# SysCV/LiDAR_snow_sim

Hardware: NVIDIA H100
Metric: augmented LiDAR points/sec (higher is better)
Workload: dtype f64

## Files before the change

### lidar_snow_sim_b200/csrc/solve.cu

```cuda
#include "beam.cuh"

namespace {

constexpr int SOLVE_TPB = 128;
constexpr int SOLVE_WARPS = SOLVE_TPB / 32;
#ifndef LSS_SOLVE_CTAS
#define LSS_SOLVE_CTAS 6
#endif
#ifndef LSS_SOLVE_ARENA
#define LSS_SOLVE_ARENA 160
#endif
constexpr int SOLVE_CTAS_PER_SM = LSS_SOLVE_CTAS;
constexpr int ARENA = LSS_SOLVE_ARENA;
constexpr int SOLVE_LCAP = 128;
static_assert(SOLVE_LCAP + 1 <= ARENA, "a beam with SOLVE_LCAP occluders must fit a round of the arena on its own");
constexpr unsigned FULL = 0xffffffffu;

struct Beam {
    double d, right, left;
    bool straddle;
};

__device__ __forceinline__ void beam_limits(float th32, double half_div, Beam &bm)
{
    const double thd = (double)th32;
    double right = thd - half_div, left = thd + half_div;
    if (right < 0) right += LSS_TWO_PI;
    if (left < 0) left += LSS_TWO_PI;
    if (right > LSS_TWO_PI) right -= LSS_TWO_PI;
    if (left > LSS_TWO_PI) left -= LSS_TWO_PI;
    bm.right = right; bm.left = left; bm.straddle = right > left;
}

__device__ __forceinline__ bool exact_hit(const ParticleRec *rp, const Beam &bm, double &rho, bool &right_hit, bool &left_hit)
{
    rho = rp->rho;
    if (!(rho < bm.d)) return false;
    const double phi = rp->phi, alpha = rp->alpha;
    bool inside = (bm.right <= phi) && (phi <= bm.left);
    if (bm.straddle) inside = inside || ((bm.right - LSS_TWO_PI <= phi) && (phi <= bm.left)) ||
                              ((bm.right <= phi) && (phi <= bm.left + LSS_TWO_PI));
    right_hit = within(bm.right - phi, alpha);
    left_hit = within(bm.left - phi, alpha);
    return inside || right_hit || left_hit;
}

struct Bucket {
    int e0, e1;
    float th_rel;
    long long pbase;
};

__device__ __forceinline__ Bucket beam_bucket(const DevArgs &a, int plane, float th32)
{
    const double thd = (double)th32;
    const double thm = thd >= LSS_TWO_PI ? thd - LSS_TWO_PI : thd;
    int bk = (int)(thm * a.inv_w);
    bk = bk < 0 ? 0 : (bk >= a.n_buckets ? a.n_buckets - 1 : bk);
    const int32_t *bs = a.bucket_start + (int64_t)plane * (a.n_buckets + 1) + bk;
    Bucket k;
    k.e0 = bs[0];
    k.e1 = bs[1];
    k.th_rel = (float)(thm - (bk + 0.5) * a.w);
    k.pbase = a.plane_off[plane];
    return k;
}

template <class F>
__device__ __forceinline__ int for_each_hit(const DevArgs &a, const Bucket &k, const Beam &bm, float d32, F &&f)
{
    int n = 0;
#pragma unroll 1
    for (int e = k.e0; e < k.e1; e++) {
        const EntryView en = lss_decode(__ldg(&a.entries[e]), a.zbase);
        if (!(en.x < d32)) break;
        if (!(fabsf(en.y - k.th_rel) <= en.z)) continue;
        const long long pi = k.pbase + en.idx;
        double rho;
        bool rh, lh;
        if (exact_hit(a.rec + pi, bm, rho, rh, lh)) { f((int)pi, rho, rh, lh); n++; }
    }
    return n;
}

constexpr int SURV_CAP = 20;

__device__ __forceinline__ double shfl_f64(double v, int src)
{
    const long long b = __double_as_longlong(v);
    const int lo = __shfl_sync(FULL, (int)(unsigned)b, src), hi = __shfl_sync(FULL, (int)(b >> 32), src);
    return __longlong_as_double(((long long)hi << 32) | (unsigned)lo);
}

#ifndef LSS_SCAN_CTAS
#define LSS_SCAN_CTAS 10
#endif
__global__ void __launch_bounds__(SNOW_TPB, LSS_SCAN_CTAS) k_scan(DevArgs a)
{
    __shared__ float s_rows[SNOW_WARPS][32 * 5];
    __shared__ int s_idx[SNOW_WARPS][32][SURV_CAP];
    __shared__ unsigned s_hit[SNOW_WARPS][32];
    const int lane = threadIdx.x & 31, wid = threadIdx.x >> 5;
    const int st = blockIdx.x * SNOW_WARPS + wid;
    if (st >= a.n_wtiles) return;
    const unsigned long long se = a.sched[st];
    const int b = (int)((se >> 32) & 0xffffu), w0 = (int)(unsigned)se;
    const int64_t beg = a.cloud_off[b];
    const int n = (int)(a.cloud_off[b + 1] - beg);
    const int i = w0 + lane;
    const bool active = i < n;
    const int nf_w = min(32, n - w0) * 5;
    float px = 0, py = 0, pz = 0, pint = 0, pch = 0;
    {
        const float *src = a.pts + (beg + w0) * 5;
#pragma unroll
        for (int q = 0; q < 5; q++) {
            const int f = q * 32 + lane;
            if (f < nf_w) s_rows[wid][f] = __ldcs(src + f);
        }
        __syncwarp();
        if (active) {
            const float *row = &s_rows[wid][5 * lane];
            px = row[0]; py = row[1]; pz = row[2]; pint = row[3]; pch = row[4];
        }
    }
    const float d32 = __fsqrt_rn(__fadd_rn(__fadd_rn(__fmul_rn(px, px), __fmul_rn(py, py)), __fmul_rn(pz, pz)));
    const int ch = channel_bin(pch);
    float out_l = pch;
    int ns = 0;
    Bucket bkt;
    bkt.e0 = bkt.e1 = 0; bkt.th_rel = 0.0f; bkt.pbase = 0;
    bool slow = false;
    float th32 = 0.0f;
    Beam bm;
    bm.d = (double)d32; bm.right = bm.left = 0.0; bm.straddle = false;
    if (active && ch < LSS_N_CHANNELS) {
        out_l = 0.0f;
        th32 = a.theta ? a.theta[beg + i] : azimuth32(py, px);
        if (th32 < 0.0f) th32 = __fadd_rn(th32, 6.2831855f);
        beam_limits(th32, a.half_div, bm);
        const int plane = a.order[b * LSS_N_CHANNELS + ch];
        if (plane >= 0 && plane < a.n_planes && th32 == th32) {
            bkt = beam_bucket(a, plane, th32);
            const int e1 = bkt.e1;
            int *pos = s_idx[wid][lane];
            bool stop = false;
#pragma unroll 1
            for (int e = bkt.e0; e < e1 && !stop; e += 4) {
                BroadEntry raw[4];
#pragma unroll
                for (int q = 0; q < 4; q++) raw[q] = __ldg(&a.entries[min(e + q, e1 - 1)]);
#pragma unroll
                for (int q = 0; q < 4; q++) {
                    if (stop || e + q >= e1) continue;
                    const EntryView en = lss_decode(raw[q], a.zbase);
                    if (!(en.x < d32)) { stop = true; continue; }
                    if (!(fabsf(en.y - bkt.th_rel) <= en.z)) continue;
                    if (ns < SURV_CAP) pos[ns] = en.idx;
                    else slow = true;
                    ns++;
                }
            }
        }
    }
    s_hit[wid][lane] = 0u;
    const int mine = slow ? 0 : ns;
    int incl = mine;
#pragma unroll
    for (int sft = 1; sft < 32; sft <<= 1) {
        const int t = __shfl_up_sync(FULL, incl, sft);
        if (lane >= sft) incl += t;
    }
    const int off = incl - mine;
    const int total = __shfl_sync(FULL, incl, 31);
    __syncwarp();
#pragma unroll 1
    for (int s0 = 0; s0 < total; s0 += 32) {
        const int s = s0 + lane;
        int j = 0;
#pragma unroll
        for (int step = 16; step; step >>= 1) {
            const int c = j + step;
            const int oc = __shfl_sync(FULL, off, c & 31);
            if (c < 32 && oc <= s) j = c;
        }
        const int r = s - __shfl_sync(FULL, off, j);
        const long long pbj = __shfl_sync(FULL, bkt.pbase, j);
        Beam bj;
        bj.d = shfl_f64(bm.d, j);
        bj.right = shfl_f64(bm.right, j);
        bj.left = shfl_f64(bm.left, j);
        bj.straddle = bj.right > bj.left;
        if (s < total) {
            double rho;
            bool rh, lh;
            if (exact_hit(a.rec + pbj + s_idx[wid][j][r], bj, rho, rh, lh)) atomicOr(&s_hit[wid][j], 1u << r);
        }
    }
    __syncwarp();
    unsigned hits = s_hit[wid][lane];
    int L = __popc(hits);
    if (slow) L = for_each_hit(a, bkt, bm, d32, [](int, double, bool, bool) {});
    {
        const bool push = L > 0;
        const unsigned pm = __ballot_sync(FULL, push);
        int lincl = push ? L : 0;
#pragma unroll
        for (int sft = 1; sft < 32; sft <<= 1) {
            const int t = __shfl_up_sync(FULL, lincl, sft);
            if (lane >= sft) lincl += t;
        }
        const int ltotal = __shfl_sync(FULL, lincl, 31);
        if (pm) {
            int hbase = 0;
            const int leader = __ffs(pm) - 1;
            if (lane == leader) hbase = atomicAdd(a.hdr + 2, ltotal);
            hbase = __shfl_sync(FULL, hbase, leader);
            if (push) {
                const int cls = LIST_CLASSES - 1 - min(LIST_CLASSES - 1, 2 * min(L, 63) + (d32 > 40.0f ? 1 : 0));
                const unsigned cm = __match_any_sync(pm, cls);
                const int cl = __ffs(cm) - 1;
                int j = 0;
                if (lane == cl) j = atomicAdd(a.hdr + LIST_CLASSES + cls, __popc(cm));
                j = __shfl_sync(cm, j, cl) + __popc(cm & ((1u << lane) - 1u));
                int *ct = a.chunk_tab + (int64_t)cls * a.chunks_per_class + j / LIST_CHUNK;
                if (j % LIST_CHUNK == 0) atomicExch(ct, atomicAdd(a.hdr, 1) + 1);
                __syncwarp(pm);
                int chunk;
                while ((chunk = *(volatile int *)ct) == 0) {}
                const int hoff = hbase + lincl - L;
                const bool fits = hoff + L <= a.hit_cap;
                {
                    SolveItem it;
                    it.key = ((unsigned long long)ch << 56) | ((unsigned long long)cls << 48) |
                             ((unsigned long long)b << 32) | (unsigned)i;
                    it.hit_off = fits ? hoff : -1;
                    it.L = L;
                    it.th32 = th32;
                    it.px = px;
                    it.py = py;
                    it.pz = pz;
                    a.items[(int64_t)(chunk - 1) * LIST_CHUNK + j % LIST_CHUNK] = it;
                }
                if (fits) {
                    int *hp = a.hit_idx + hoff;
                    if (!slow) {
                        const int *pos = s_idx[wid][lane];
#pragma unroll 1
                        for (int k = 0; hits; hits &= hits - 1) hp[k++] = (int)bkt.pbase + pos[__ffs(hits) - 1];
                    } else {
                        for_each_hit(a, bkt, bm, d32, [&](int pi, double, bool, bool) { *hp++ = pi; });
                    }
                }
            }
        }
    }
    __syncwarp();
    if (active) {
        float *row = &s_rows[wid][5 * lane];
        const float out_i = rintf(pint);
        row[3] = out_i;
        row[4] = out_l;
        if (a.nocc) a.nocc[beg + i] = 0;
        a.keep_d[beg + i] = d32;
        a.keep_i[beg + i] = out_i;
        a.keep_tag[beg + i] = (uint8_t)ch;
    }
    __syncwarp();
    {
        float *dst = a.aug + (beg + w0) * 5;
#pragma unroll
        for (int q = 0; q < 5; q++) {
            const int f = q * 32 + lane;
            if (f < nf_w) dst[f] = s_rows[wid][f];
        }
    }
}

__device__ __forceinline__ unsigned long long pack_win(int ks, int ke, int k0)
{
    return (unsigned long long)(unsigned)ks | ((unsigned long long)(unsigned)ke << 11) | ((unsigned long long)(unsigned)k0 << 22);
}

__device__ __forceinline__ void pulse_phase(double r, double &sb, double &cb)
{
    const double ctau = 299792458.0 * 1e-8, inv_ctau = 1.0 / (299792458.0 * 1e-8);
    const double bh = r * inv_ctau;
    const double bl = fma(-bh, ctau, r) * inv_ctau;
    double s, c;
    sincospi(bh, &s, &c);
    const double corr = LSS_PI * bl;
    sb = fma(corr, c, s);
    cb = fma(-corr, s, c);
}

__global__ void __launch_bounds__(SOLVE_TPB, SOLVE_CTAS_PER_SM) k_solve(DevArgs a, int *tile_cursor)
{
    __shared__ double s_arena[SOLVE_WARPS][4][ARENA];
    __shared__ unsigned long long s_piece[SOLVE_WARPS][2 * ARENA];
    __shared__ int s_piece_k[SOLVE_WARPS][2 * ARENA];
    const int lane = threadIdx.x & 31, wid = threadIdx.x >> 5;
    unsigned long long *PD = s_piece[wid];
    int *PK = s_piece_k[wid];
    double *A0 = s_arena[wid][0], *A1 = s_arena[wid][1], *A2 = s_arena[wid][2], *A3 = s_arena[wid][3];
    unsigned long long *W = reinterpret_cast<unsigned long long *>(A2);

    __shared__ int s_tile0[LIST_CLASSES + 1];
    const int *cls_cnt = a.hdr + LIST_CLASSES;
    if (wid == 0) {
        int run = 0;
        for (int c0 = 0; c0 < LIST_CLASSES; c0 += 32) {
            const int v = (cls_cnt[c0 + lane] + 31) >> 5;
            int incl = v;
#pragma unroll
            for (int sft = 1; sft < 32; sft <<= 1) {
                const int t = __shfl_up_sync(FULL, incl, sft);
                if (lane >= sft) incl += t;
            }
            s_tile0[c0 + lane] = run + incl - v;
            run += __shfl_sync(FULL, incl, 31);
        }
        if (lane == 0) s_tile0[LIST_CLASSES] = run;
    }
    __syncthreads();
    const int n_tiles = s_tile0[LIST_CLASSES];
    const double ctau = 299792458.0 * 1e-8;
    const double inv_step = (double)(LSS_M_EXT - 1) / (120 + ctau);

    for (;;) {
        int tile = 0;
        if (lane == 0) tile = atomicAdd(tile_cursor, 1);
        tile = __shfl_sync(FULL, tile, 0);
        if (tile >= n_tiles) break;
        int cls = 0;
#pragma unroll
        for (int step = LIST_CLASSES / 2; step; step >>= 1)
            if (s_tile0[cls + step] <= tile) cls += step;
        const int j = (tile - s_tile0[cls]) * 32 + lane;
        const bool active = j < cls_cnt[cls];
        SolveItem it;
        it.key = 0ull; it.hit_off = 0; it.L = 0; it.th32 = 0.0f; it.px = 0.0f; it.py = 0.0f; it.pz = 0.0f;
        if (active) {
            const int chunk = a.chunk_tab[(int64_t)cls * a.chunks_per_class + j / LIST_CHUNK];
            it = a.items[(int64_t)(chunk - 1) * LIST_CHUNK + j % LIST_CHUNK];
        }
        const int b = (int)((it.key >> 32) & 0xffffu);
        const int i = (int)(it.key & 0xffffffffu);
        const int ch = (int)(it.key >> 56);
        const int64_t beg = a.cloud_off[b];
        const float px = it.px, py = it.py, pz = it.pz;
        const float d32 = __fsqrt_rn(__fadd_rn(__fadd_rn(__fmul_rn(px, px), __fmul_rn(py, py)), __fmul_rn(pz, pz)));

        float out_x = px, out_y = py, out_z = pz, out_i = 0.0f, out_l = 0.0f;
        long long att_new_i = -1;
        int n_claim = 0;

        const int L = active ? it.L : 0;
        Beam bm;
        bm.d = (double)d32;
        beam_limits(it.th32, a.half_div, bm);

        if (L > SOLVE_LCAP) raise_status(a.status, LSS_ERR_OCCLUDER_OVERFLOW);
        const int need = (L > 0 && L <= SOLVE_LCAP) ? L + 1 : 0;

        unsigned remaining = __ballot_sync(FULL, need > 0);
        while (remaining) {
            const bool rem = (remaining >> lane) & 1u;
            const int mine = rem ? need : 0;
            int incl = mine;
#pragma unroll
            for (int s = 1; s < 32; s <<= 1) {
                const int t = __shfl_up_sync(FULL, incl, s);
                if (lane >= s) incl += t;
            }
            const bool in_round = rem && incl <= ARENA;
            remaining &= ~__ballot_sync(FULL, in_round);
            const int off = incl - mine;
            const int total = (int)__reduce_max_sync(FULL, in_round ? (unsigned)incl : 0u);
            int n_pulses = 0;
            double amax = 0.0;
            double best = 0.0;
            int kbest = 0;

#pragma unroll 1
            for (int s0 = 0; s0 < total; s0 += 32) {
                const int s = s0 + lane;
                int j = 0;
#pragma unroll
                for (int step = 16; step; step >>= 1) {
                    const int c = j + step;
                    const int oc = __shfl_sync(FULL, off, c & 31);
                    if (c < 32 && oc <= s) j = c;
                }
                const int r = s - __shfl_sync(FULL, off, j);
                const int Lj = __shfl_sync(FULL, L, j);
                const int hoj = __shfl_sync(FULL, it.hit_off, j);
                const int inr = __shfl_sync(FULL, (int)in_round, j);
                Beam bj;
                bj.d = shfl_f64(bm.d, j);
                bj.right = shfl_f64(bm.right, j);
                bj.left = shfl_f64(bm.left, j);
                bj.straddle = bj.right > bj.left;
                if (s < total && inr && r < Lj && hoj >= 0) {
                    const int pi = a.hit_idx[hoj + r];
                    const ParticleTan tn = a.tan[pi];
                    double rho;
                    bool rh, lh;
                    exact_hit(a.rec + pi, bj, rho, rh, lh);
                    A0[s] = rh ? bj.right : tn.t_right;
                    A1[s] = lh ? bj.left : tn.t_left;
                    A2[s] = rho;
                }
            }
            if (in_round && it.hit_off < 0) {
                const Bucket bkt = beam_bucket(a, a.order[b * LSS_N_CHANNELS + ch], it.th32);
                int s = off;
                for_each_hit(a, bkt, bm, d32, [&](int pi, double rho, bool rh, bool lh) {
                    A0[s] = rh ? bm.right : a.tan[pi].t_right;
                    A1[s] = lh ? bm.left : a.tan[pi].t_left;
                    A2[s] = rho;
                    s++;
                });
            }
            __syncwarp();

            if (in_round) {
#pragma unroll 1
                for (int p = 1; p < L; p++) {
                    const double rho = A2[off + p];
                    if (!(A2[off + p - 1] > rho)) continue;
                    const double a1 = A0[off + p], a2 = A1[off + p];
                    int q = p - 1;
#pragma unroll 1
                    while (q >= 0 && A2[off + q] > rho) { A0[off + q + 1] = A0[off + q]; A1[off + q + 1] = A1[off + q]; A2[off + q + 1] = A2[off + q]; q--; }
                    A0[off + q + 1] = a1; A1[off + q + 1] = a2; A2[off + q + 1] = rho;
                }

                double rb = bm.right;
                if (bm.straddle) rb = bm.right - LSS_TWO_PI;
                int nu = 0, P = 0;
                double ep_min = fmin(rb, bm.left), ep_max = fmax(rb, bm.left), claimed_total = 0.0;
#pragma unroll 1
                for (int j = 0; j < L; j++) {
                    double lo = A0[off + j];
                    const double hi = A1[off + j], rho = A2[off + j];
                    if (bm.straddle && lo > hi) lo -= LSS_TWO_PI;
                    ep_min = fmin(ep_min, fmin(lo, hi));
                    ep_max = fmax(ep_max, fmax(lo, hi));
                    if (!(lo < hi)) continue;
                    bool contained = false;
                    double cov = 0.0, nlo = lo, nhi = hi;
                    int w = 0;
#pragma unroll 1
                    for (int u = 0; u < nu; u++) {
                        const double ul = A0[off + u], uh = A1[off + u];
                        if ((ul <= lo) && (hi <= uh)) { contained = true; break; }
                        if (ul <= hi && uh >= lo) {
                            const double ov = fmin(hi, uh) - fmax(lo, ul);
                            if (ov > 0.0) cov += ov;
                            nlo = fmin(nlo, ul);
                            nhi = fmax(nhi, uh);
                        } else {
                            A0[off + w] = ul; A1[off + w] = uh; w++;
                        }
                    }
                    if (contained) continue;
                    const double claimed = (hi - lo) - cov;
                    claimed_total += claimed;
                    A0[off + w] = nlo; A1[off + w] = nhi;
                    nu = w + 1;
                    double ratio = claimed / a.div_rad;
                    ratio = ratio < 0 ? 0 : (ratio > 1 ? 1 : ratio);
                    A2[off + P] = rho;
                    A3[off + P] = ratio;
                    P++;
                }
                n_claim = P;
                double ratio_hard = ((ep_max - ep_min) - claimed_total) / a.div_rad;
                ratio_hard = ratio_hard < 0 ? 0 : (ratio_hard > 1 ? 1 : ratio_hard);

                if (P > 0) {
                    const double beta_0 = 1 * 1e-06 / LSS_PI;
                    const double i_orig = 0.9 * a.sensor->max_intensity[ch];
                    const double A = (i_orig / beta_0) * beta_0;
                    bool bad = false;
#pragma unroll 1
                    for (int j = 0; j < P; j++) {
                        const double r = A2[off + j], ratio = A3[off + j];
                        const int ks = (int)ceil(r * 10);
                        const int ke = (int)(floor((r + ctau) * 10) + 1);
                        bad |= (ke > LSS_M_EXT) || (ks < 0);
                        double sb, cb;
                        pulse_phase(r, sb, cb);
                        const double amp = (A * ratio * xsi64(r)) / (r * r);
                        amax = fmax(amax, amp);
                        A0[off + j] = amp;
                        A1[off + j] = sb;
                        A3[off + j] = cb;
                        W[off + j] = pack_win(ks, ke, (int)rint((r + ctau / 2) * inv_step));
                    }
                    {
                        const int ks = (int)ceilf(__fmul_rn(d32, 10.0f));
                        const int ke = (int)(floorf(__fmul_rn(__fadd_rn(d32, (float)ctau), 10.0f)) + 1.0f);
                        bad |= (ke > LSS_M_EXT) || (ks < 0);
                        double sb, cb;
                        pulse_phase(bm.d, sb, cb);
                        const double amp = (A * ratio_hard * xsi32(d32)) / (double)__fmul_rn(d32, d32);
                        amax = fmax(amax, amp);
                        A0[off + P] = amp;
                        A1[off + P] = sb;
                        A3[off + P] = cb;
                        W[off + P] = pack_win(ks, ke, (int)rint((bm.d + ctau / 2) * inv_step));
                    }
                    if (bad) raise_status(a.status, LSS_ERR_RANGE_INDEX);
                    else n_pulses = P + 1;
                }
            }

            int np_mine = 0;
            if (n_pulses > 0) {
                const double lb = 0.99 * amax;
                double asum = 0.0;
                int qa = 0, qb = -1, nxt = 0;
                int ks_n = (int)(W[off] & 2047u);
                int ke_a = 0;
                int k = ks_n;
                unsigned long long *pd = PD + 2 * off;
#pragma unroll 1
                for (;;) {
#pragma unroll 1
                    while (ks_n <= k) {
                        qb = nxt++;
                        asum += A0[off + qb];
                        ks_n = nxt < n_pulses ? (int)(W[off + nxt] & 2047u) : 4096;
                    }
#pragma unroll 1
                    while (qa <= qb) {
                        ke_a = (int)((W[off + qa] >> 11) & 2047u);
                        if (ke_a > k) break;
                        asum -= A0[off + qa];
                        qa++;
                    }
                    if (qa > qb) {
                        asum = 0.0;
                        if (nxt >= n_pulses) break;
                        k = ks_n;
                        continue;
                    }
                    const int pend = min(ke_a, ks_n);
                    if (asum * 1.0001 >= lb)
                        pd[np_mine++] = (unsigned long long)(unsigned)k | ((unsigned long long)(unsigned)pend << 11) |
                                        ((unsigned long long)(unsigned)(off + qa) << 22) | ((unsigned long long)(unsigned)(off + qb) << 32);
                    k = pend;
                }
            }
            int pincl = np_mine;
#pragma unroll
            for (int sft = 1; sft < 32; sft <<= 1) {
                const int t = __shfl_up_sync(FULL, pincl, sft);
                if (lane >= sft) pincl += t;
            }
            const int pex = pincl - np_mine;
            const int ptotal = __shfl_sync(FULL, pincl, 31);
            __syncwarp();
            {
                const float step = (float)((120 + ctau) / (double)(LSS_M_EXT - 1));
                const float ctau_f = (float)ctau;
#pragma unroll 1
                for (int f0 = 0; f0 < ptotal; f0 += 32) {
                    const int f = f0 + lane;
                    int j = 0;
#pragma unroll
                    for (int stp = 16; stp; stp >>= 1) {
                        const int c = j + stp;
                        const int oc = __shfl_sync(FULL, pex, c & 31);
                        if (c < 32 && oc <= f) j = c;
                    }
                    const int slot = 2 * __shfl_sync(FULL, off, j) + (f - __shfl_sync(FULL, pex, j));
                    if (f < ptotal) {
                        const unsigned long long d = PD[slot];
                        const int lo = (int)(d & 2047u), hi = (int)((d >> 11) & 2047u);
                        const int qa = (int)((d >> 22) & 1023u), qb = (int)((d >> 32) & 1023u);
                        double pbest = 0.0;
                        int pk = lo;
                        auto eval = [&](int c) {
                            const double2 t = __ldg(&a.wtab[c]);
                            double v = 0.0;
#pragma unroll 1
                            for (int q = qa; q <= qb; q++) {
                                const double sn = t.x * A3[q] - t.y * A1[q];
                                v += A0[q] * (sn * sn);
                            }
                            if (v > pbest) { pbest = v; pk = c; }
                        };
                        int kc;
                        bool all = false;
                        if (qa == qb) {
                            kc = (int)((W[qa] >> 22) & 2047u);
                        } else {
                            float zx = 0.0f, zy = 0.0f, asum = 0.0f;
#pragma unroll 1
                            for (int q = qa; q <= qb; q++) {
                                const float A = (float)A0[q], sn = (float)A1[q], cs = (float)A3[q];
                                zx += A * (cs * cs - sn * sn);
                                zy += A * (2.0f * sn * cs);
                                asum += A;
                            }
                            all = zx * zx + zy * zy < 1e-6f * asum * asum;
                            const float r0 = (atan2f(zy, zx) + 3.14159265f) * (ctau_f * 0.15915494f);
                            const float rc = 0.5f * (float)(lo + hi - 1) * step;
                            kc = (int)rintf((r0 + rintf((rc - r0) / ctau_f) * ctau_f) / step);
                        }
                        const int c_lo = all ? lo : max(lo, min(hi - 1, kc - 1));
                        const int c_hi = all ? hi - 1 : min(hi - 1, max(lo, kc + 1));
#pragma unroll 1
                        for (int c = c_lo; c <= c_hi; c++) eval(c);
                        PD[slot] = (unsigned long long)__double_as_longlong(pbest);
                        PK[slot] = pk;
                    }
                }
            }
            __syncwarp();
#pragma unroll 1
            for (int r = 0; r < np_mine; r++) {
                const double v = __longlong_as_double((long long)PD[2 * off + r]);
                if (v > best) { best = v; kbest = PK[2 * off + r]; }
            }
            __syncwarp();

            if (n_pulses > 0) {
                const double max_i = a.sensor->max_intensity[ch];
                const double min_i = a.sensor->min_intensity[ch];
                const double d_max = ((double)kbest / 10) - (ctau / 2);
                const double q1 = 1 - d_max / 120;
                double i_max = best + max_i * a.sensor->focal_slope[ch] * fabs(a.sensor->focal_offset[ch] - q1 * q1);
                i_max = i_max < min_i ? min_i : (i_max > max_i ? max_i : i_max);
                const long long new_i = (long long)i_max;
                if (fabs(d_max - bm.d) < 2 * (1.0 / 10)) {
                    out_l = 1.0f;
                    att_new_i = new_i;
                } else {
                    out_l = 2.0f;
                    const double sc = d_max / bm.d;
                    out_x = (float)((double)px * sc);
                    out_y = (float)((double)py * sc);
                    out_z = (float)((double)pz * sc);
                }
                if (new_i < 0) raise_status(a.status, LSS_ERR_NEGATIVE_INTENSITY);
                double ci = (double)new_i;
                ci = ci < min_i ? min_i : (ci > max_i ? max_i : ci);
                out_i = (float)ci;
            }
            __syncwarp();
        }

        if (active) {
            if (out_l != 0.0f) {
                const float ri = rintf(out_i);
                float *row = a.aug + (beg + i) * 5;
                row[0] = out_x; row[1] = out_y; row[2] = out_z; row[3] = ri; row[4] = out_l;
                a.keep_i[beg + i] = ri;
                a.keep_tag[beg + i] = keep_tag_of(ch, out_l);
            }
            if (a.nocc) a.nocc[beg + i] = n_claim;
        }
        {
            const bool on = att_new_i >= 0;
            const int key = b * LSS_N_CHANNELS + (ch < LSS_N_CHANNELS ? ch : 0);
            const unsigned mk = __match_any_sync(FULL, on ? key : -1);
            if (on && lane == __ffs(mk) - 1) atomicAdd(a.att_cnt + key, (unsigned)__popc(mk));
            const unsigned mb = __match_any_sync(FULL, on ? b : -1);
            const unsigned sum = __reduce_add_sync(mb, on ? (unsigned)att_new_i : 0u);
            if (on && lane == __ffs(mb) - 1) atomicAdd(&a.att_sum[b], (unsigned long long)sum);
        }
    }
}

}

namespace {
__global__ void k_debug_azimuth(const float *y, const float *x, float *out, int64_t n)
{
    const int64_t i = (int64_t)blockIdx.x * blockDim.x + threadIdx.x;
    if (i < n) out[i] = azimuth32(y[i], x[i]);
}
}

extern "C" lss_status lss_debug_azimuth(lss_engine *e, const float *d_y, const float *d_x, int64_t n, float *d_out, void *stream)
{
    if (!e || !d_y || !d_x || !d_out || n < 0) return LSS_ERR_INVALID_ARG;
    if (n == 0) return LSS_OK;
    DeviceGuard g(e->device);
    LSS_CUDA_CHECK(e, lss_launch(e, k_debug_azimuth, (unsigned)((n + 255) / 256), 256, 0, (cudaStream_t)stream, d_y, d_x,
                                 d_out, n));
    return LSS_OK;
}

cudaError_t lss_launch_scan(lss_engine *e, const DevArgs &a, cudaStream_t stream)
{
    return lss_launch(e, k_scan, (unsigned)((a.n_wtiles + SNOW_WARPS - 1) / SNOW_WARPS), SNOW_TPB, 0, stream, a);
}

cudaError_t lss_launch_solve(lss_engine *e, const DevArgs &a, int *tile_cursor, cudaStream_t stream)
{
    return lss_launch(e, k_solve, (unsigned)(e->n_sm * SOLVE_CTAS_PER_SM), SOLVE_TPB, 0, stream, a, tile_cursor);
}
```

Baseline: 4.158 billion.

## Batch arena fill gathers with cp.async and make exact_hit branchless

The arena fill loop in k_solve now works in two passes. The first resolves all owner lanes and particle indices up front. The second issues cp.async 8-byte copies of the tangent and particle-record fields straight into shared memory, then waits once and evaluates the hit test from shared. Together these put many independent global gathers in flight at once instead of one dependent chain per 32-slot round. exact_hit now takes a preloaded record and folds the range test into its result without an early return. The scan kernel also shuffles 32-bit pbase and the float distance instead of 64-bit values. The costs are extra registers for the unrolled index arrays and the reuse of A3/PD as staging space. Widening the float d32 to double for bj.d in the scan could also change boundary hit results slightly.

```diff
diff --git a/lidar_snow_sim_b200/csrc/solve.cu b/lidar_snow_sim_b200/csrc/solve.cu
--- a/lidar_snow_sim_b200/csrc/solve.cu
+++ b/lidar_snow_sim_b200/csrc/solve.cu
@@ -32,17 +32,25 @@
     bm.right = right; bm.left = left; bm.straddle = right > left;
 }
 
-__device__ __forceinline__ bool exact_hit(const ParticleRec *rp, const Beam &bm, double &rho, bool &right_hit, bool &left_hit)
-{
-    rho = rp->rho;
-    if (!(rho < bm.d)) return false;
-    const double phi = rp->phi, alpha = rp->alpha;
+__device__ __forceinline__ ParticleRec load_rec(const ParticleRec *rp)
+{
+    ParticleRec p;
+    p.phi = rp->phi;
+    p.rho = rp->rho;
+    p.alpha = rp->alpha;
+    return p;
+}
+
+__device__ __forceinline__ bool exact_hit(const ParticleRec &p, const Beam &bm, bool &right_hit, bool &left_hit)
+{
+    const bool nearer = p.rho < bm.d;
+    const double phi = p.phi, alpha = p.alpha;
     bool inside = (bm.right <= phi) && (phi <= bm.left);
     if (bm.straddle) inside = inside || ((bm.right - LSS_TWO_PI <= phi) && (phi <= bm.left)) ||
                               ((bm.right <= phi) && (phi <= bm.left + LSS_TWO_PI));
     right_hit = within(bm.right - phi, alpha);
     left_hit = within(bm.left - phi, alpha);
-    return inside || right_hit || left_hit;
+    return nearer & (inside || right_hit || left_hit);
 }
 
 struct Bucket {
@@ -76,9 +84,9 @@
         if (!(en.x < d32)) break;
         if (!(fabsf(en.y - k.th_rel) <= en.z)) continue;
         const long long pi = k.pbase + en.idx;
-        double rho;
+        const ParticleRec p = load_rec(a.rec + pi);
         bool rh, lh;
-        if (exact_hit(a.rec + pi, bm, rho, rh, lh)) { f((int)pi, rho, rh, lh); n++; }
+        if (exact_hit(p, bm, rh, lh)) { f((int)pi, p.rho, rh, lh); n++; }
     }
     return n;
 }
@@ -185,16 +193,15 @@
             if (c < 32 && oc <= s) j = c;
         }
         const int r = s - __shfl_sync(FULL, off, j);
-        const long long pbj = __shfl_sync(FULL, bkt.pbase, j);
+        const int pbj = __shfl_sync(FULL, (int)bkt.pbase, j);
         Beam bj;
-        bj.d = shfl_f64(bm.d, j);
+        bj.d = (double)__shfl_sync(FULL, d32, j);
         bj.right = shfl_f64(bm.right, j);
         bj.left = shfl_f64(bm.left, j);
         bj.straddle = bj.right > bj.left;
         if (s < total) {
-            double rho;
             bool rh, lh;
-            if (exact_hit(a.rec + pbj + s_idx[wid][j][r], bj, rho, rh, lh)) atomicOr(&s_hit[wid][j], 1u << r);
+            if (exact_hit(load_rec(a.rec + pbj + s_idx[wid][j][r]), bj, rh, lh)) atomicOr(&s_hit[wid][j], 1u << r);
         }
     }
     __syncwarp();
@@ -294,6 +301,17 @@
     cb = fma(-corr, s, c);
 }
 
+__device__ __forceinline__ void cp_async8(void *dst_shared, const void *src_global)
+{
+    asm volatile("cp.async.ca.shared.global [%0], [%1], 8;\n" ::"r"((unsigned)__cvta_generic_to_shared(dst_shared)),
+                 "l"(src_global) : "memory");
+}
+
+__device__ __forceinline__ void cp_async_wait_all() { asm volatile("cp.async.wait_all;\n" ::: "memory"); }
+
+constexpr int FILL_K = (ARENA + 31) / 32;
+static_assert(6 * FILL_K <= 32, "the fill keeps 6 bits per slot of a lane (owner lane, filled) in one register");
+
 __global__ void __launch_bounds__(SOLVE_TPB, SOLVE_CTAS_PER_SM) k_solve(DevArgs a, int *tile_cursor)
 {
     __shared__ double s_arena[SOLVE_WARPS][4][ARENA];
@@ -382,34 +400,63 @@
             double best = 0.0;
             int kbest = 0;
 
-#pragma unroll 1
-            for (int s0 = 0; s0 < total; s0 += 32) {
-                const int s = s0 + lane;
-                int j = 0;
-#pragma unroll
-                for (int step = 16; step; step >>= 1) {
-                    const int c = j + step;
-                    const int oc = __shfl_sync(FULL, off, c & 31);
-                    if (c < 32 && oc <= s) j = c;
-                }
-                const int r = s - __shfl_sync(FULL, off, j);
-                const int Lj = __shfl_sync(FULL, L, j);
-                const int hoj = __shfl_sync(FULL, it.hit_off, j);
-                const int inr = __shfl_sync(FULL, (int)in_round, j);
-                Beam bj;
-                bj.d = shfl_f64(bm.d, j);
-                bj.right = shfl_f64(bm.right, j);
-                bj.left = shfl_f64(bm.left, j);
-                bj.straddle = bj.right > bj.left;
-                if (s < total && inr && r < Lj && hoj >= 0) {
-                    const int pi = a.hit_idx[hoj + r];
-                    const ParticleTan tn = a.tan[pi];
-                    double rho;
-                    bool rh, lh;
-                    exact_hit(a.rec + pi, bj, rho, rh, lh);
-                    A0[s] = rh ? bj.right : tn.t_right;
-                    A1[s] = lh ? bj.left : tn.t_left;
-                    A2[s] = rho;
+            int pidx[FILL_K];
+            unsigned owners = 0;
+#pragma unroll
+            for (int k = 0; k < FILL_K; k++) {
+                pidx[k] = 0;
+                if (32 * k < total) {
+                    const int s = 32 * k + lane;
+                    int j = 0;
+#pragma unroll
+                    for (int step = 16; step; step >>= 1) {
+                        const int c = j + step;
+                        const int oc = __shfl_sync(FULL, off, c & 31);
+                        if (c < 32 && oc <= s) j = c;
+                    }
+                    const int r = s - __shfl_sync(FULL, off, j);
+                    const int Lj = __shfl_sync(FULL, L, j);
+                    const int hoj = __shfl_sync(FULL, it.hit_off, j);
+                    const int inr = __shfl_sync(FULL, (int)in_round, j);
+                    const bool fill = s < total && inr && r < Lj && hoj >= 0;
+                    if (fill) pidx[k] = a.hit_idx[hoj + r];
+                    owners |= (unsigned)(j | (fill ? 32 : 0)) << (6 * k);
+                }
+            }
+#pragma unroll
+            for (int k = 0; k < FILL_K; k++) {
+                if ((owners >> (6 * k + 5)) & 1u) {
+                    const int s = 32 * k + lane;
+                    const ParticleRec *rp = a.rec + pidx[k];
+                    const ParticleTan *tp = a.tan + pidx[k];
+                    cp_async8(&A0[s], &tp->t_right);
+                    cp_async8(&A1[s], &tp->t_left);
+                    cp_async8(&A2[s], &rp->rho);
+                    cp_async8(&A3[s], &rp->phi);
+                    cp_async8(&PD[s], &rp->alpha);
+                }
+            }
+            cp_async_wait_all();
+#pragma unroll
+            for (int k = 0; k < FILL_K; k++) {
+                if (32 * k < total) {
+                    const int j = (owners >> (6 * k)) & 31u;
+                    Beam bj;
+                    bj.d = shfl_f64(bm.d, j);
+                    bj.right = shfl_f64(bm.right, j);
+                    bj.left = shfl_f64(bm.left, j);
+                    bj.straddle = bj.right > bj.left;
+                    if ((owners >> (6 * k + 5)) & 1u) {
+                        const int s = 32 * k + lane;
+                        ParticleRec p;
+                        p.phi = A3[s];
+                        p.rho = A2[s];
+                        p.alpha = __longlong_as_double((long long)PD[s]);
+                        bool rh, lh;
+                        exact_hit(p, bj, rh, lh);
+                        if (rh) A0[s] = bj.right;
+                        if (lh) A1[s] = bj.left;
+                    }
                 }
             }
             if (in_round && it.hit_off < 0) {
```

Result: faster. 4.257 billion (median of 6 runs) (+2.4%).
